# songweige/rich-text-to-image

Hardware: NVIDIA H100
Metric: denoising steps/sec (higher is better)
Workload: dtype f16

## Files before the change

### rich-text-to-image_b200/csrc/gemm_geglu.cu

```cuda
#include "ptx.cuh"
#include "rtti_internal.h"

namespace rtti {
namespace gg {
constexpr int BM = 128, BN = 128, BK = 64;
constexpr int STAGES = 4;
constexpr int A_TILE = BM * BK * 2;
constexpr int B_TILE = 2 * BN * BK * 2;
constexpr int STAGE = A_TILE + B_TILE;
constexpr int OFF_BAR = STAGES * STAGE;
constexpr int SMEM_BYTES = OFF_BAR + 64 + 1024;
constexpr int THREADS = 256;
}

struct GegluParams {
  const __half* bias;
  __half* y;
  int M, N, K;
  int n_blocks, k_blocks;
};

__device__ __forceinline__ float gelu_erf(float x) { return 0.5f * x * (1.f + erff(x * 0.70710678118654752f)); }

__global__ void __launch_bounds__(gg::THREADS, 1)
ff_geglu_kernel(const __grid_constant__ CUtensorMap tm_a, const __grid_constant__ CUtensorMap tm_b,
                const __grid_constant__ GegluParams p) {
  using namespace gg;
  extern __shared__ uint8_t smem_raw[];
  uint8_t* smem = reinterpret_cast<uint8_t*>((reinterpret_cast<uintptr_t>(smem_raw) + 1023) & ~uintptr_t(1023));
  uint64_t* full = reinterpret_cast<uint64_t*>(smem + OFF_BAR);

  const int tid = threadIdx.x, wg = tid >> 7, w = (tid >> 5) & 3, lane = tid & 31;
  const int m0 = (blockIdx.x / p.n_blocks) * BM, n0 = (blockIdx.x % p.n_blocks) * BN;

  auto load = [&](int kb) {
    const int s = kb % STAGES;
    uint8_t* st = smem + s * STAGE;
    mbar_expect_tx(&full[s], STAGE);
    tma_load_2d(st, &tm_a, &full[s], kb * BK, m0);
    tma_load_2d(st + A_TILE, &tm_b, &full[s], kb * BK, n0);
    tma_load_2d(st + A_TILE + B_TILE / 2, &tm_b, &full[s], kb * BK, p.N + n0);
  };
  if (tid == 0) {
    tma_prefetch_desc(&tm_a); tma_prefetch_desc(&tm_b);
    for (int i = 0; i < STAGES; ++i) mbar_init(&full[i], 1);
    mbar_fence_init();
    for (int kb = 0; kb < STAGES && kb < p.k_blocks; ++kb) load(kb);
  }
  __syncthreads();

  const uint32_t sbase = smem_u32(smem);
  float v[64], g[64];
  for (int kb = 0; kb < p.k_blocks; ++kb) {
    const int s = kb % STAGES;
    const uint32_t aa = sbase + s * STAGE + wg * 64 * 128;
    const uint32_t ba = sbase + s * STAGE + A_TILE;
    mbar_wait(&full[s], (kb / STAGES) & 1);
    wgmma_fence();
#pragma unroll
    for (int kk = 0; kk < BK / 16; ++kk) {
      const uint64_t da = wgmma_desc_sw128(aa + kk * 32, 16, 1024);
      const uint32_t acc = (kb > 0 || kk > 0) ? 1u : 0u;
      wgmma_ss<128>(v, da, wgmma_desc_sw128(ba + kk * 32, 16, 1024), acc);
      wgmma_ss<128>(g, da, wgmma_desc_sw128(ba + B_TILE / 2 + kk * 32, 16, 1024), acc);
    }
    wgmma_commit();
    wgmma_wait_all<64>(v);
    pin_regs<64>(g);
    __syncthreads();
    if (tid == 0 && kb + STAGES < p.k_blocks) load(kb + STAGES);
  }

  const int r0 = m0 + 64 * wg + 16 * w + (lane >> 2), r1 = r0 + 8;
  const int cq = 2 * (lane & 3);
#pragma unroll
  for (int i = 0; i < 16; ++i) {
    const int col = n0 + 8 * i + cq;
    float2 bv = make_float2(0.f, 0.f), bg = make_float2(0.f, 0.f);
    if (p.bias != nullptr) {
      bv = __half22float2(*reinterpret_cast<const __half2*>(p.bias + col));
      bg = __half22float2(*reinterpret_cast<const __half2*>(p.bias + p.N + col));
    }
    if (r0 < p.M)
      *reinterpret_cast<__half2*>(p.y + static_cast<size_t>(r0) * p.N + col) =
          __floats2half2_rn((v[4 * i] + bv.x) * gelu_erf(g[4 * i] + bg.x), (v[4 * i + 1] + bv.y) * gelu_erf(g[4 * i + 1] + bg.y));
    if (r1 < p.M)
      *reinterpret_cast<__half2*>(p.y + static_cast<size_t>(r1) * p.N + col) =
          __floats2half2_rn((v[4 * i + 2] + bv.x) * gelu_erf(g[4 * i + 2] + bg.x), (v[4 * i + 3] + bv.y) * gelu_erf(g[4 * i + 3] + bg.y));
  }
}

static int make_2d_map(CUtensorMap* m, const void* ptr, long long rows, long long cols, long long row_stride_elems,
                       int box_rows) {
  cuuint64_t dims[2] = {(cuuint64_t)cols, (cuuint64_t)rows};
  cuuint64_t strides[1] = {(cuuint64_t)row_stride_elems * 2};
  cuuint32_t box[2] = {64, (cuuint32_t)box_rows};
  cuuint32_t estr[2] = {1, 1};
  return encode_tiled_f16(m, ptr, 2, dims, strides, box, estr);
}

}

using namespace rtti;

extern "C" int rtti_ff_geglu_fwd(const void* x, const void* w, const void* bias, void* y, long long m, int n, int k,
                                 void* stream) {
  if (!x || !w || !y) return RTTI_ERR_ARG;
  if (m < 1 || n < 1 || k < 1) return RTTI_ERR_ARG;
  if (n % gg::BN != 0 || k % gg::BK != 0) return RTTI_ERR_SHAPE;
  if (((uintptr_t)x | (uintptr_t)w | (uintptr_t)y | (uintptr_t)bias) & 15) return RTTI_ERR_ALIGN;
  int rc = rtti_arch_ok();
  if (rc != RTTI_OK) return rc;
  CUtensorMap ta, tb;
  if ((rc = make_2d_map(&ta, x, m, k, k, gg::BM)) != RTTI_OK) return rc;
  if ((rc = make_2d_map(&tb, w, 2LL * n, k, k, gg::BN)) != RTTI_OK) return rc;
  static const bool configured =
      cudaFuncSetAttribute(ff_geglu_kernel, cudaFuncAttributeMaxDynamicSharedMemorySize, gg::SMEM_BYTES) == cudaSuccess;
  if (!configured) return RTTI_ERR_CUDA;
  GegluParams p{};
  p.bias = (const __half*)bias; p.y = (__half*)y; p.M = (int)m; p.N = n; p.K = k;
  p.n_blocks = n / gg::BN; p.k_blocks = k / gg::BK;
  const long long tiles = ((m + gg::BM - 1) / gg::BM) * p.n_blocks;
  if (tiles > 0x7fffffffLL) return RTTI_ERR_SHAPE;
  ff_geglu_kernel<<<(unsigned)tiles, gg::THREADS, gg::SMEM_BYTES, (cudaStream_t)stream>>>(ta, tb, p);
  return cudaGetLastError() == cudaSuccess ? RTTI_OK : RTTI_ERR_CUDA;
}
```

### rich-text-to-image_b200/csrc/ptx.cuh

```cuda
#pragma once
#include <cuda.h>
#include <cuda_fp16.h>
#include <cuda_runtime.h>
#include <stdint.h>

namespace rtti {

__device__ __forceinline__ uint32_t smem_u32(const void* p) {
  return static_cast<uint32_t>(__cvta_generic_to_shared(p));
}

__device__ __forceinline__ void mbar_init(uint64_t* bar, uint32_t count) {
  asm volatile("mbarrier.init.shared::cta.b64 [%0], %1;\n" ::"r"(smem_u32(bar)), "r"(count));
}
__device__ __forceinline__ void mbar_fence_init() {
  asm volatile("fence.mbarrier_init.release.cluster;\n" ::: "memory");
}
__device__ __forceinline__ void mbar_expect_tx(uint64_t* bar, uint32_t bytes) {
  asm volatile("mbarrier.arrive.expect_tx.shared::cta.b64 _, [%0], %1;\n" ::"r"(smem_u32(bar)),
               "r"(bytes)
               : "memory");
}
__device__ __forceinline__ void mbar_arrive(uint64_t* bar) {
  asm volatile("mbarrier.arrive.shared::cta.b64 _, [%0];\n" ::"r"(smem_u32(bar)) : "memory");
}
__device__ __forceinline__ void mbar_wait(uint64_t* bar, uint32_t parity) {
  asm volatile(
      "{\n\t.reg .pred P1;\n\t"
      "WAIT_LOOP:\n\t"
      "mbarrier.try_wait.parity.shared::cta.b64 P1, [%0], %1;\n\t"
      "@P1 bra.uni WAIT_DONE;\n\t"
      "bra.uni WAIT_LOOP;\n\t"
      "WAIT_DONE:\n\t}\n" ::"r"(smem_u32(bar)),
      "r"(parity)
      : "memory");
}

__device__ __forceinline__ void tma_prefetch_desc(const CUtensorMap* m) {
  asm volatile("prefetch.tensormap [%0];\n" ::"l"(reinterpret_cast<uint64_t>(m)) : "memory");
}
__device__ __forceinline__ void tma_load_4d(void* smem_dst, const CUtensorMap* m, uint64_t* bar, int c0,
                                            int c1, int c2, int c3) {
  asm volatile(
      "cp.async.bulk.tensor.4d.shared::cluster.global.mbarrier::complete_tx::bytes"
      " [%0], [%1, {%3, %4, %5, %6}], [%2];\n" ::"r"(smem_u32(smem_dst)),
      "l"(reinterpret_cast<uint64_t>(m)), "r"(smem_u32(bar)), "r"(c0), "r"(c1), "r"(c2), "r"(c3)
      : "memory");
}
__device__ __forceinline__ void tma_store_4d(const CUtensorMap* m, const void* smem_src, int c0, int c1,
                                             int c2, int c3) {
  asm volatile(
      "cp.async.bulk.tensor.4d.global.shared::cta.bulk_group [%0, {%2, %3, %4, %5}], [%1];\n" ::"l"(
          reinterpret_cast<uint64_t>(m)),
      "r"(smem_u32(smem_src)), "r"(c0), "r"(c1), "r"(c2), "r"(c3)
      : "memory");
}
__device__ __forceinline__ void tma_store_commit() { asm volatile("cp.async.bulk.commit_group;\n" ::: "memory"); }
__device__ __forceinline__ void tma_store_wait_read() {
  asm volatile("cp.async.bulk.wait_group.read 0;\n" ::: "memory");
}
__device__ __forceinline__ void tma_store_wait_all() {
  asm volatile("cp.async.bulk.wait_group 0;\n" ::: "memory");
}
__device__ __forceinline__ void fence_proxy_async_smem() {
  asm volatile("fence.proxy.async.shared::cta;\n" ::: "memory");
}

__device__ __forceinline__ void tma_load_2d(void* smem_dst, const CUtensorMap* m, uint64_t* bar, int c0, int c1) {
  asm volatile(
      "cp.async.bulk.tensor.2d.shared::cluster.global.mbarrier::complete_tx::bytes"
      " [%0], [%1, {%3, %4}], [%2];\n" ::"r"(smem_u32(smem_dst)),
      "l"(reinterpret_cast<uint64_t>(m)), "r"(smem_u32(bar)), "r"(c0), "r"(c1)
      : "memory");
}

__device__ __forceinline__ uint64_t wgmma_desc_sw128(uint32_t smem_addr, uint32_t lbo_bytes, uint32_t sbo_bytes) {
  uint64_t d = 0;
  d |= static_cast<uint64_t>((smem_addr & 0x3FFFF) >> 4);
  d |= static_cast<uint64_t>((lbo_bytes >> 4) & 0x3FFF) << 16;
  d |= static_cast<uint64_t>((sbo_bytes >> 4) & 0x3FFF) << 32;
  d |= static_cast<uint64_t>(1) << 62;
  return d;
}

__device__ __forceinline__ void wgmma_fence() { asm volatile("wgmma.fence.sync.aligned;\n" ::: "memory"); }
__device__ __forceinline__ void wgmma_commit() { asm volatile("wgmma.commit_group.sync.aligned;\n" ::: "memory"); }
template <int N>
__device__ __forceinline__ void wgmma_wait_all(float* d) {
  asm volatile("wgmma.wait_group.sync.aligned 0;\n" ::: "memory");
#pragma unroll
  for (int i = 0; i < N; ++i) asm volatile("" : "+f"(d[i])::"memory");
}
template <int N>
__device__ __forceinline__ void pin_regs(float* d) {
#pragma unroll
  for (int i = 0; i < N; ++i) asm volatile("" : "+f"(d[i])::"memory");
}

template <int N> __device__ __forceinline__ void wgmma_ss(float* d, uint64_t da, uint64_t db, uint32_t acc);
template <int N> __device__ __forceinline__ void wgmma_rs_tb(float* d, const uint32_t* a, uint64_t db, uint32_t acc);
template <> __device__ __forceinline__ void wgmma_ss<64>(float* d, uint64_t da, uint64_t db, uint32_t acc) {
  asm volatile(
      "{\n\t.reg .pred p;\n\tsetp.ne.b32 p, %34, 0;\n\t"
      "wgmma.mma_async.sync.aligned.m64n64k16.f32.f16.f16 {%0, %1, %2, %3, %4, %5, %6, %7, %8, %9, %10, %11, %12, %13, %14, %15, %16, %17, %18, %19, %20, %21, %22, %23, %24, %25, %26, %27, %28, %29, %30, %31}, %32, %33, p, 1, 1, 0, 0;\n\t}\n"
      : "+f"(d[0]), "+f"(d[1]), "+f"(d[2]), "+f"(d[3]), "+f"(d[4]), "+f"(d[5]), "+f"(d[6]), "+f"(d[7]), "+f"(d[8]), "+f"(d[9]), "+f"(d[10]), "+f"(d[11]), "+f"(d[12]), "+f"(d[13]), "+f"(d[14]), "+f"(d[15]), "+f"(d[16]), "+f"(d[17]), "+f"(d[18]), "+f"(d[19]), "+f"(d[20]), "+f"(d[21]), "+f"(d[22]), "+f"(d[23]), "+f"(d[24]), "+f"(d[25]), "+f"(d[26]), "+f"(d[27]), "+f"(d[28]), "+f"(d[29]), "+f"(d[30]), "+f"(d[31])
      : "l"(da), "l"(db), "r"(acc));
}

template <> __device__ __forceinline__ void wgmma_ss<80>(float* d, uint64_t da, uint64_t db, uint32_t acc) {
  asm volatile(
      "{\n\t.reg .pred p;\n\tsetp.ne.b32 p, %42, 0;\n\t"
      "wgmma.mma_async.sync.aligned.m64n80k16.f32.f16.f16 {%0, %1, %2, %3, %4, %5, %6, %7, %8, %9, %10, %11, %12, %13, %14, %15, %16, %17, %18, %19, %20, %21, %22, %23, %24, %25, %26, %27, %28, %29, %30, %31, %32, %33, %34, %35, %36, %37, %38, %39}, %40, %41, p, 1, 1, 0, 0;\n\t}\n"
      : "+f"(d[0]), "+f"(d[1]), "+f"(d[2]), "+f"(d[3]), "+f"(d[4]), "+f"(d[5]), "+f"(d[6]), "+f"(d[7]), "+f"(d[8]), "+f"(d[9]), "+f"(d[10]), "+f"(d[11]), "+f"(d[12]), "+f"(d[13]), "+f"(d[14]), "+f"(d[15]), "+f"(d[16]), "+f"(d[17]), "+f"(d[18]), "+f"(d[19]), "+f"(d[20]), "+f"(d[21]), "+f"(d[22]), "+f"(d[23]), "+f"(d[24]), "+f"(d[25]), "+f"(d[26]), "+f"(d[27]), "+f"(d[28]), "+f"(d[29]), "+f"(d[30]), "+f"(d[31]), "+f"(d[32]), "+f"(d[33]), "+f"(d[34]), "+f"(d[35]), "+f"(d[36]), "+f"(d[37]), "+f"(d[38]), "+f"(d[39])
      : "l"(da), "l"(db), "r"(acc));
}

template <> __device__ __forceinline__ void wgmma_ss<128>(float* d, uint64_t da, uint64_t db, uint32_t acc) {
  asm volatile(
      "{\n\t.reg .pred p;\n\tsetp.ne.b32 p, %66, 0;\n\t"
      "wgmma.mma_async.sync.aligned.m64n128k16.f32.f16.f16 {%0, %1, %2, %3, %4, %5, %6, %7, %8, %9, %10, %11, %12, %13, %14, %15, %16, %17, %18, %19, %20, %21, %22, %23, %24, %25, %26, %27, %28, %29, %30, %31, %32, %33, %34, %35, %36, %37, %38, %39, %40, %41, %42, %43, %44, %45, %46, %47, %48, %49, %50, %51, %52, %53, %54, %55, %56, %57, %58, %59, %60, %61, %62, %63}, %64, %65, p, 1, 1, 0, 0;\n\t}\n"
      : "+f"(d[0]), "+f"(d[1]), "+f"(d[2]), "+f"(d[3]), "+f"(d[4]), "+f"(d[5]), "+f"(d[6]), "+f"(d[7]), "+f"(d[8]), "+f"(d[9]), "+f"(d[10]), "+f"(d[11]), "+f"(d[12]), "+f"(d[13]), "+f"(d[14]), "+f"(d[15]), "+f"(d[16]), "+f"(d[17]), "+f"(d[18]), "+f"(d[19]), "+f"(d[20]), "+f"(d[21]), "+f"(d[22]), "+f"(d[23]), "+f"(d[24]), "+f"(d[25]), "+f"(d[26]), "+f"(d[27]), "+f"(d[28]), "+f"(d[29]), "+f"(d[30]), "+f"(d[31]), "+f"(d[32]), "+f"(d[33]), "+f"(d[34]), "+f"(d[35]), "+f"(d[36]), "+f"(d[37]), "+f"(d[38]), "+f"(d[39]), "+f"(d[40]), "+f"(d[41]), "+f"(d[42]), "+f"(d[43]), "+f"(d[44]), "+f"(d[45]), "+f"(d[46]), "+f"(d[47]), "+f"(d[48]), "+f"(d[49]), "+f"(d[50]), "+f"(d[51]), "+f"(d[52]), "+f"(d[53]), "+f"(d[54]), "+f"(d[55]), "+f"(d[56]), "+f"(d[57]), "+f"(d[58]), "+f"(d[59]), "+f"(d[60]), "+f"(d[61]), "+f"(d[62]), "+f"(d[63])
      : "l"(da), "l"(db), "r"(acc));
}

template <> __device__ __forceinline__ void wgmma_rs_tb<64>(float* d, const uint32_t* a, uint64_t db, uint32_t acc) {
  asm volatile(
      "{\n\t.reg .pred p;\n\tsetp.ne.b32 p, %37, 0;\n\t"
      "wgmma.mma_async.sync.aligned.m64n64k16.f32.f16.f16 {%0, %1, %2, %3, %4, %5, %6, %7, %8, %9, %10, %11, %12, %13, %14, %15, %16, %17, %18, %19, %20, %21, %22, %23, %24, %25, %26, %27, %28, %29, %30, %31}, {%32, %33, %34, %35}, %36, p, 1, 1, 1;\n\t}\n"
      : "+f"(d[0]), "+f"(d[1]), "+f"(d[2]), "+f"(d[3]), "+f"(d[4]), "+f"(d[5]), "+f"(d[6]), "+f"(d[7]), "+f"(d[8]), "+f"(d[9]), "+f"(d[10]), "+f"(d[11]), "+f"(d[12]), "+f"(d[13]), "+f"(d[14]), "+f"(d[15]), "+f"(d[16]), "+f"(d[17]), "+f"(d[18]), "+f"(d[19]), "+f"(d[20]), "+f"(d[21]), "+f"(d[22]), "+f"(d[23]), "+f"(d[24]), "+f"(d[25]), "+f"(d[26]), "+f"(d[27]), "+f"(d[28]), "+f"(d[29]), "+f"(d[30]), "+f"(d[31])
      : "r"(a[0]), "r"(a[1]), "r"(a[2]), "r"(a[3]), "l"(db), "r"(acc));
}

__device__ __forceinline__ float ex2_approx(float x) {
  float y;
  asm("ex2.approx.ftz.f32 %0, %1;\n" : "=f"(y) : "f"(x));
  return y;
}
__device__ __forceinline__ uint32_t pack_half2(float lo, float hi) {
  __half2 h = __floats2half2_rn(lo, hi);
  return *reinterpret_cast<uint32_t*>(&h);
}

}
```

### rich-text-to-image_b200/unet.py

```python
import math
from dataclasses import dataclass, field
from typing import Dict, List, Optional, Tuple

import torch
import torch.nn as nn
import torch.nn.functional as F

from . import ops

FEATURE_INJECT_RESNET = "up_blocks.1.resnets.1"


@dataclass
class UNetConfig:
    sample_size: int = 64
    in_channels: int = 4
    out_channels: int = 4
    down_block_types: Tuple[str, ...] = ("CrossAttnDownBlock2D", "CrossAttnDownBlock2D", "CrossAttnDownBlock2D", "DownBlock2D")
    up_block_types: Tuple[str, ...] = ("UpBlock2D", "CrossAttnUpBlock2D", "CrossAttnUpBlock2D", "CrossAttnUpBlock2D")
    block_out_channels: Tuple[int, ...] = (320, 640, 1280, 1280)
    layers_per_block: int = 2
    transformer_layers_per_block: Tuple[int, ...] = (1, 1, 1, 1)
    attention_head_dim: Tuple[int, ...] = (8, 8, 8, 8)
    cross_attention_dim: int = 768
    use_linear_projection: bool = False
    addition_embed_type: Optional[str] = None
    addition_time_embed_dim: Optional[int] = None
    projection_class_embeddings_input_dim: Optional[int] = None
    norm_num_groups: int = 32
    norm_eps: float = 1e-5
    flip_sin_to_cos: bool = True
    freq_shift: int = 0

    @staticmethod
    def sd15():
        return UNetConfig()

    @staticmethod
    def sdxl():
        return UNetConfig(sample_size=128, down_block_types=("DownBlock2D", "CrossAttnDownBlock2D", "CrossAttnDownBlock2D"),
                          up_block_types=("CrossAttnUpBlock2D", "CrossAttnUpBlock2D", "UpBlock2D"),
                          block_out_channels=(320, 640, 1280), transformer_layers_per_block=(1, 2, 10),
                          attention_head_dim=(5, 10, 20), cross_attention_dim=2048, use_linear_projection=True,
                          addition_embed_type="text_time", addition_time_embed_dim=256,
                          projection_class_embeddings_input_dim=2816)

    @staticmethod
    def from_dict(d):
        keys = UNetConfig.__dataclass_fields__.keys()
        kw = {k: (tuple(v) if isinstance(v, list) else v) for k, v in d.items() if k in keys}
        n = len(kw.get("block_out_channels", (0,) * 4))
        for k in ("transformer_layers_per_block", "attention_head_dim"):
            if k in kw and isinstance(kw[k], int):
                kw[k] = (kw[k],) * n
        return UNetConfig(**kw)


class TokenMapAccumulator:

    def __init__(self, cross_layers, self_layers=None, start_after=10, sd_overwrite_bug=False,
                 self_resolutions=(32,)):
        self.cross_layers = set(cross_layers)
        self.self_layers = None if self_layers is None else set(self_layers)
        self.start_after = start_after
        self.sd_overwrite_bug = sd_overwrite_bug
        self.self_resolutions = None if self_resolutions is None else set(self_resolutions)
        self.selfattn_maps: Dict[str, torch.Tensor] = {}
        self.crossattn_maps: Dict[str, torch.Tensor] = {}
        self.n_maps: Dict[str, int] = {}

    def tick(self, name):
        self.n_maps[name] = self.n_maps.get(name, 0) + 1
        return self.n_maps[name] > self.start_after

    def cross_target(self, name, n_q, n_k, device):
        if not self.tick(name) or name not in self.cross_layers:
            return None
        if name not in self.crossattn_maps:
            self.crossattn_maps[name] = torch.zeros(1, n_q, n_k, dtype=torch.float32, device=device)
        return self.crossattn_maps[name]

    def self_target(self, name, n_q, device):
        if not self.tick(name):
            return None
        if self.self_layers is not None and name not in self.self_layers:
            return None
        if self.self_resolutions is not None and int(round(math.sqrt(n_q))) not in self.self_resolutions:
            return None
        if name not in self.selfattn_maps:
            self.selfattn_maps[name] = torch.zeros(1, n_q, n_q, dtype=torch.float32, device=device)
        elif self.sd_overwrite_bug and name not in self.crossattn_maps:
            self.selfattn_maps[name].zero_()
        return self.selfattn_maps[name]


class CrossKVCache:

    def __init__(self):
        self.kv: Dict[str, torch.Tensor] = {}


@dataclass
class RegionControl:
    qk_src: Optional[List[int]] = None
    feature_src: Optional[List[int]] = None
    feature_idx: Optional[torch.Tensor] = None
    word_pos: Optional[torch.Tensor] = None
    font_size: Optional[torch.Tensor] = None
    fs_batch_mask: int = 0
    capture: Optional[TokenMapAccumulator] = None
    capture_row: int = 1
    kv_cache: Optional[CrossKVCache] = None
    remote: Optional[object] = None


def _f16(t):
    return t.to(torch.float16)


class GroupNormCL(nn.Module):

    def __init__(self, groups, channels, eps):
        super().__init__()
        self.groups, self.eps = groups, eps
        self.weight = nn.Parameter(torch.ones(channels))
        self.bias = nn.Parameter(torch.zeros(channels))

    def forward(self, x, silu, chan_bias=None):
        return ops.groupnorm_silu(x, self.weight, self.bias, self.groups, self.eps, silu, chan_bias=chan_bias)


class LayerNormCL(nn.Module):
    def __init__(self, channels, eps=1e-5):
        super().__init__()
        self.eps = eps
        self.weight = nn.Parameter(torch.ones(channels))
        self.bias = nn.Parameter(torch.zeros(channels))

    def forward(self, x):
        return ops.layernorm(x, self.weight, self.bias, self.eps)


class Conv2dCL(nn.Conv2d):

    def forward_cl(self, x, H, W, with_bias=True):
        B = x.shape[0]
        x4 = x.view(B, H, W, -1).permute(0, 3, 1, 2)
        y = F.conv2d(x4, self.weight, self.bias if with_bias else None, self.stride, self.padding)
        Ho, Wo = y.shape[2], y.shape[3]
        y = y.permute(0, 2, 3, 1)
        if not y.is_contiguous():
            y = y.contiguous()
        return y.reshape(B, Ho * Wo, -1), Ho, Wo


class Attention(nn.Module):

    def __init__(self, query_dim, cross_attention_dim, heads):
        super().__init__()
        self.heads = heads
        self.is_cross = cross_attention_dim is not None
        kv_dim = cross_attention_dim if self.is_cross else query_dim
        self.to_q = nn.Linear(query_dim, query_dim, bias=False)
        self.to_k = nn.Linear(kv_dim, query_dim, bias=False)
        self.to_v = nn.Linear(kv_dim, query_dim, bias=False)
        self.to_out = nn.ModuleList([nn.Linear(query_dim, query_dim)])
        self._fused = None

    def fused_weight(self):
        ver = (self.to_k.weight._version, self.to_v.weight._version, self.to_q.weight._version,
               self.to_k.weight.data_ptr(), self.to_k.weight.dtype)
        if self._fused is None or self._fused[0] != ver:
            ws = [self.to_k.weight, self.to_v.weight] if self.is_cross else [self.to_q.weight, self.to_k.weight, self.to_v.weight]
            self._fused = (ver, torch.cat([w.detach() for w in ws], 0).contiguous())
        return self._fused[1]


class BasicTransformerBlock(nn.Module):
    def __init__(self, dim, heads, cross_attention_dim):
        super().__init__()
        self.norm1 = LayerNormCL(dim)
        self.attn1 = Attention(dim, None, heads)
        self.norm2 = LayerNormCL(dim)
        self.attn2 = Attention(dim, cross_attention_dim, heads)
        self.norm3 = LayerNormCL(dim)
        self.ff = nn.Module()
        self.ff.net = nn.ModuleList([nn.Module(), nn.Identity(), nn.Linear(dim * 4, dim)])
        self.ff.net[0].proj = nn.Linear(dim, dim * 8)

    def forward(self, h, n, ctx, ctrl: RegionControl, name):
        B, T, C = h.shape
        heads = self.attn1.heads
        cap = ctrl.capture
        rem = ctrl.remote
        if rem is not None and rem.is_dst:
            k0 = rem.n_own
            w3 = self.attn1.fused_weight()
            o = torch.empty(B, T, C, dtype=h.dtype, device=h.device)
            if k0:
                qkv = F.linear(n[:k0], w3)
                ops.attention(qkv[..., :C], qkv[..., C:2 * C], qkv[..., 2 * C:], heads, out=o[:k0])
            v = F.linear(n[k0:], w3[2 * C:])
            rqk = rem.wait(T, 2 * C)
            ops.attention(rqk[..., :C], rqk[..., C:], v, heads, qk_src=[0] * (B - k0), out=o[k0:])
        else:
            qkv = F.linear(n, self.attn1.fused_weight())
            q, k, v = qkv[..., :C], qkv[..., C:2 * C], qkv[..., 2 * C:]
            if rem is not None and rem.is_src:
                rem.push(qkv[rem.d_index, :, :2 * C])
            tgt = cap.self_target(name + ".attn1", T, h.device) if cap is not None else None
            lse = torch.empty(B, heads, T, dtype=torch.float32, device=h.device) if tgt is not None else None
            o = ops.attention(q, k, v, heads, qk_src=ctrl.qk_src, lse=lse)
            if tgt is not None:
                r = ctrl.capture_row
                ops.attn_probs_mean_accum(q[r], k[r], lse[r], tgt[0], heads)
        a = F.linear(o, self.attn1.to_out[0].weight)
        h, n = ops.add_bias_layernorm(a, h, self.attn1.to_out[0].bias, self.norm2.weight, self.norm2.bias, self.norm2.eps)
        q = F.linear(n, self.attn2.to_q.weight)
        kv = None
        key = name + ".attn2"
        if ctrl.kv_cache is not None:
            kv = ctrl.kv_cache.kv.get(key)
        if kv is None:
            kv = F.linear(ctx, self.attn2.fused_weight())
            if ctrl.kv_cache is not None:
                ctrl.kv_cache.kv[key] = kv
        ck, cv = kv[..., :C], kv[..., C:]
        pbar, slots = None, None
        if cap is not None:
            pbar = cap.cross_target(key, T, ctx.shape[1], h.device)
            if pbar is not None:
                slots = [-1] * B
                slots[ctrl.capture_row] = 0
        o = ops.attention(q, ck, cv, heads, word_pos=ctrl.word_pos, font_size=ctrl.font_size,
                          fs_batch_mask=ctrl.fs_batch_mask, pbar_accum=pbar, cap_slot=slots)
        a = F.linear(o, self.attn2.to_out[0].weight)
        h, n = ops.add_bias_layernorm(a, h, self.attn2.to_out[0].bias, self.norm3.weight, self.norm3.bias, self.norm3.eps)
        proj = self.ff.net[0].proj
        if ops.FUSED_FF_GEGLU and C % 64 == 0:
            g = ops.ff_geglu(n, proj.weight, proj.bias)
        else:
            g = ops.geglu(F.linear(n, proj.weight, proj.bias))
        a = F.linear(g, self.ff.net[2].weight)
        if rem is not None and rem.is_src:
            rem.join()
            del qkv
        return h, a, self.ff.net[2].bias


class Transformer2DModel(nn.Module):
    def __init__(self, channels, heads, layers, cross_attention_dim, groups, use_linear_projection):
        super().__init__()
        self.use_linear_projection = use_linear_projection
        self.norm = GroupNormCL(groups, channels, 1e-6)
        if use_linear_projection:
            self.proj_in = nn.Linear(channels, channels)
            self.proj_out = nn.Linear(channels, channels)
        else:
            self.proj_in = nn.Conv2d(channels, channels, 1)
            self.proj_out = nn.Conv2d(channels, channels, 1)
        self.transformer_blocks = nn.ModuleList([BasicTransformerBlock(channels, heads, cross_attention_dim) for _ in range(layers)])

    def _proj(self, mod, x):
        w = mod.weight if self.use_linear_projection else mod.weight.view(mod.weight.shape[0], -1)
        return F.linear(x, w, mod.bias)

    def forward(self, x, ctx, ctrl, name):
        h = self.norm(x, silu=False)
        h = self._proj(self.proj_in, h)
        blocks = self.transformer_blocks
        n = blocks[0].norm1(h)
        for i, blk in enumerate(blocks):
            h, a, bias = blk(h, n, ctx, ctrl, f"{name}.transformer_blocks.{i}")
            if i + 1 < len(blocks):
                nxt = blocks[i + 1].norm1
                h, n = ops.add_bias_layernorm(a, h, bias, nxt.weight, nxt.bias, nxt.eps)
            else:
                h = ops.add_bias_f16(h, a, bias, out=a)
        w = self.proj_out.weight if self.use_linear_projection else self.proj_out.weight.view(self.proj_out.weight.shape[0], -1)
        y = F.linear(h, w)
        return ops.add_bias_f16(x, y, self.proj_out.bias, out=y)


class ResnetBlock2D(nn.Module):
    def __init__(self, cin, cout, temb_ch, groups, eps):
        super().__init__()
        self.norm1 = GroupNormCL(groups, cin, eps)
        self.conv1 = Conv2dCL(cin, cout, 3, padding=1)
        self.time_emb_proj = nn.Linear(temb_ch, cout)
        self.norm2 = GroupNormCL(groups, cout, eps)
        self.conv2 = Conv2dCL(cout, cout, 3, padding=1)
        self.conv_shortcut = nn.Conv2d(cin, cout, 1) if cin != cout else None

    def forward(self, x, H, W, temb_act, feature_idx=None, remote=None):
        h = self.norm1(x, silu=True)
        h, _, _ = self.conv1.forward_cl(h, H, W, with_bias=False)
        t = F.linear(temb_act, self.time_emb_proj.weight, self.time_emb_proj.bias + self.conv1.bias)
        h = self.norm2(h, silu=True, chan_bias=t.contiguous())
        h, _, _ = self.conv2.forward_cl(h, H, W, with_bias=False)
        if remote is not None and remote.is_src:
            remote.push(h[remote.d_index])
            remote.join()
        if remote is not None and remote.is_dst:
            f = remote.wait(h.shape[1], h.shape[2])
            h = torch.cat([h[:remote.n_own], f.expand(h.shape[0] - remote.n_own, -1, -1)], 0)
        elif feature_idx is not None:
            h = h.index_select(0, feature_idx)
        if self.conv_shortcut is not None:
            x = F.linear(x, self.conv_shortcut.weight.view(self.conv_shortcut.weight.shape[0], -1), self.conv_shortcut.bias)
        return ops.add_bias_f16(x, h, self.conv2.bias, out=h)


class Downsample2D(nn.Module):
    def __init__(self, ch):
        super().__init__()
        self.conv = Conv2dCL(ch, ch, 3, stride=2, padding=1)


class Upsample2D(nn.Module):
    def __init__(self, ch):
        super().__init__()
        self.conv = Conv2dCL(ch, ch, 3, padding=1)

    def forward(self, x, H, W):
        B, _, C = x.shape
        x = x.view(B, H, 1, W, 1, C).expand(B, H, 2, W, 2, C).reshape(B, 4 * H * W, C)
        return self.conv.forward_cl(x, 2 * H, 2 * W)


class _Block(nn.Module):
    pass


class UNet2DConditionModel(nn.Module):
    def __init__(self, cfg: UNetConfig):
        super().__init__()
        self.config = cfg
        self.in_channels = cfg.in_channels
        boc = cfg.block_out_channels
        temb = boc[0] * 4
        g, eps = cfg.norm_num_groups, cfg.norm_eps
        self.conv_in = Conv2dCL(cfg.in_channels, boc[0], 3, padding=1)
        self.time_embedding = nn.Module()
        self.time_embedding.linear_1 = nn.Linear(boc[0], temb)
        self.time_embedding.linear_2 = nn.Linear(temb, temb)
        if cfg.addition_embed_type == "text_time":
            self.add_embedding = nn.Module()
            self.add_embedding.linear_1 = nn.Linear(cfg.projection_class_embeddings_input_dim, temb)
            self.add_embedding.linear_2 = nn.Linear(temb, temb)
        self.down_blocks = nn.ModuleList()
        out_c = boc[0]
        for i, typ in enumerate(cfg.down_block_types):
            in_c, out_c = out_c, boc[i]
            blk = _Block()
            blk.has_cross_attention = typ == "CrossAttnDownBlock2D"
            if blk.has_cross_attention:
                blk.attentions = nn.ModuleList([
                    Transformer2DModel(out_c, cfg.attention_head_dim[i], cfg.transformer_layers_per_block[i],
                                       cfg.cross_attention_dim, g, cfg.use_linear_projection)
                    for _ in range(cfg.layers_per_block)])
            blk.resnets = nn.ModuleList([ResnetBlock2D(in_c if l == 0 else out_c, out_c, temb, g, eps)
                                         for l in range(cfg.layers_per_block)])
            if i != len(boc) - 1:
                blk.downsamplers = nn.ModuleList([Downsample2D(out_c)])
            else:
                blk.downsamplers = None
            self.down_blocks.append(blk)
        self.mid_block = _Block()
        self.mid_block.attentions = nn.ModuleList([
            Transformer2DModel(boc[-1], cfg.attention_head_dim[-1], cfg.transformer_layers_per_block[-1],
                               cfg.cross_attention_dim, g, cfg.use_linear_projection)])
        self.mid_block.resnets = nn.ModuleList([ResnetBlock2D(boc[-1], boc[-1], temb, g, eps) for _ in range(2)])
        self.up_blocks = nn.ModuleList()
        rev = list(reversed(boc))
        rev_heads = list(reversed(cfg.attention_head_dim))
        rev_layers = list(reversed(cfg.transformer_layers_per_block))
        out_c = rev[0]
        for i, typ in enumerate(cfg.up_block_types):
            prev, out_c = out_c, rev[i]
            in_c = rev[min(i + 1, len(boc) - 1)]
            n = cfg.layers_per_block + 1
            blk = _Block()
            blk.has_cross_attention = typ == "CrossAttnUpBlock2D"
            if blk.has_cross_attention:
                blk.attentions = nn.ModuleList([
                    Transformer2DModel(out_c, rev_heads[i], rev_layers[i], cfg.cross_attention_dim, g, cfg.use_linear_projection)
                    for _ in range(n)])
            blk.resnets = nn.ModuleList([
                ResnetBlock2D((prev if l == 0 else out_c) + (in_c if l == n - 1 else out_c), out_c, temb, g, eps)
                for l in range(n)])
            blk.upsamplers = nn.ModuleList([Upsample2D(out_c)]) if i != len(boc) - 1 else None
            self.up_blocks.append(blk)
        self.conv_norm_out = GroupNormCL(g, boc[0], eps)
        self.conv_out = Conv2dCL(boc[0], cfg.out_channels, 3, padding=1)

    def injection_layout(self, H, W):
        out = []

        def attn(tr, H, W):
            C = tr.proj_in.weight.shape[0]
            out.extend([(H * W, 2 * C)] * len(tr.transformer_blocks))

        for i, blk in enumerate(self.down_blocks):
            for l in range(len(blk.resnets)):
                if blk.has_cross_attention:
                    attn(blk.attentions[l], H, W)
            if blk.downsamplers is not None:
                H, W = (H + 1) // 2, (W + 1) // 2
        attn(self.mid_block.attentions[0], H, W)
        for i, blk in enumerate(self.up_blocks):
            for l, res in enumerate(blk.resnets):
                if f"up_blocks.{i}.resnets.{l}" == FEATURE_INJECT_RESNET:
                    out.append((H * W, res.conv2.weight.shape[0]))
                if blk.has_cross_attention:
                    attn(blk.attentions[l], H, W)
            if blk.upsamplers is not None:
                H, W = 2 * H, 2 * W
        return out

    def finalize(self, device="cuda"):
        self.to(device=device, dtype=torch.float16)
        for m in self.modules():
            if isinstance(m, nn.Conv2d) and m.kernel_size != (1, 1):
                m.weight.data = m.weight.data.contiguous(memory_format=torch.channels_last)
        self.requires_grad_(False)
        return self.eval()

    def init_synthetic(self, seed=0):
        g = torch.Generator(device=self.conv_in.weight.device).manual_seed(seed)
        for name, p in self.named_parameters():
            if p.dim() >= 2:
                fan_in = p[0].numel()
                p.data.copy_(torch.randn(p.shape, generator=g, device=p.device, dtype=torch.float32) / math.sqrt(fan_in))
            elif name.endswith("weight"):
                p.data.fill_(1.0)
            else:
                p.data.copy_(0.05 * torch.randn(p.shape, generator=g, device=p.device, dtype=torch.float32))
        return self

    def _timestep_embedding(self, t, dim, device):
        half = dim // 2
        exponent = -math.log(10000) * torch.arange(half, dtype=torch.float32, device=device) / (half - self.config.freq_shift)
        emb = t[:, None].float() * torch.exp(exponent)[None, :]
        emb = torch.cat([torch.sin(emb), torch.cos(emb)], dim=-1)
        if self.config.flip_sin_to_cos:
            emb = torch.cat([emb[:, half:], emb[:, :half]], dim=-1)
        return emb

    def forward(self, sample, timestep, encoder_hidden_states, added_cond_kwargs=None, ctrl: Optional[RegionControl] = None,
                return_dict=True, **unused):
        cfg = self.config
        ctrl = ctrl or RegionControl()
        dev = sample.device
        B, _, H, W = sample.shape
        t = torch.as_tensor(timestep, device=dev)
        if t.dim() == 0:
            t = t[None]
        t = t.expand(B)
        mlp = lambda m, x: F.linear(F.silu(F.linear(x, m.linear_1.weight, m.linear_1.bias)), m.linear_2.weight, m.linear_2.bias)
        emb = mlp(self.time_embedding, _f16(self._timestep_embedding(t, cfg.block_out_channels[0], dev)))
        if cfg.addition_embed_type == "text_time":
            time_ids = added_cond_kwargs["time_ids"].to(dev)
            te = self._timestep_embedding(time_ids.flatten(), cfg.addition_time_embed_dim, dev)
            te = te.reshape(time_ids.shape[0], -1)
            if te.shape[0] != B:
                te = te[:1].expand(B, -1)
            add = torch.cat([_f16(added_cond_kwargs["text_embeds"]), _f16(te)], dim=-1)
            emb = emb + mlp(self.add_embedding, add)
        temb_act = F.silu(emb)
        ctx = _f16(encoder_hidden_states).contiguous()
        feat_idx = ctrl.feature_idx
        if feat_idx is None and ctrl.feature_src is not None:
            feat_idx = torch.as_tensor(ctrl.feature_src, device=dev)

        x = _f16(sample).permute(0, 2, 3, 1).contiguous().view(B, H * W, -1)
        h, H, W = self.conv_in.forward_cl(x, H, W)
        skips = [(h, H, W)]
        for i, blk in enumerate(self.down_blocks):
            for l, res in enumerate(blk.resnets):
                h = res(h, H, W, temb_act)
                if blk.has_cross_attention:
                    h = blk.attentions[l](h, ctx, ctrl, f"down_blocks.{i}.attentions.{l}")
                skips.append((h, H, W))
            if blk.downsamplers is not None:
                h, H, W = blk.downsamplers[0].conv.forward_cl(h, H, W)
                skips.append((h, H, W))
        h = self.mid_block.resnets[0](h, H, W, temb_act)
        h = self.mid_block.attentions[0](h, ctx, ctrl, "mid_block.attentions.0")
        h = self.mid_block.resnets[1](h, H, W, temb_act)
        for i, blk in enumerate(self.up_blocks):
            for l, res in enumerate(blk.resnets):
                s, _, _ = skips.pop()
                h = torch.cat([h, s], dim=-1)
                rname = f"up_blocks.{i}.resnets.{l}"
                inj = rname == FEATURE_INJECT_RESNET
                h = res(h, H, W, temb_act, feat_idx if inj else None, ctrl.remote if inj else None)
                if blk.has_cross_attention:
                    h = blk.attentions[l](h, ctx, ctrl, f"up_blocks.{i}.attentions.{l}")
            if blk.upsamplers is not None:
                h, H, W = blk.upsamplers[0](h, H, W)
        h = self.conv_norm_out(h, silu=True)
        h, H, W = self.conv_out.forward_cl(h, H, W)
        out = h.view(B, H, W, -1).permute(0, 3, 1, 2).contiguous()
        return {"sample": out} if return_dict else (out,)
```

Measured before the change: 4.810.

## Warp-specialize persistent GEGLU GEMM and skip redundant QK projections in self-attention

The GEGLU feed-forward GEMM becomes a persistent, warp-specialized kernel. One producer warpgroup issues TMA loads through full/empty mbarriers while two consumer warpgroups each run m64n256 wgmma over both value and gate halves, with register reallocation via setmaxnreg. Tiles are swizzled in groups along M for L2 reuse, and outputs are staged in shared memory and written with TMA stores. Separately, the UNet self-attention path now computes only V for batch rows whose Q/K come from an earlier row and reuses that row's QK. This cuts GEMM work but adds control logic and shape assumptions.

```diff
diff --git a/rich-text-to-image_b200/csrc/gemm_geglu.cu b/rich-text-to-image_b200/csrc/gemm_geglu.cu
--- a/rich-text-to-image_b200/csrc/gemm_geglu.cu
+++ b/rich-text-to-image_b200/csrc/gemm_geglu.cu
@@ -5,89 +5,128 @@
 namespace gg {
 constexpr int BM = 128, BN = 128, BK = 64;
 constexpr int STAGES = 4;
+constexpr int GROUP_M = 8;
 constexpr int A_TILE = BM * BK * 2;
 constexpr int B_TILE = 2 * BN * BK * 2;
 constexpr int STAGE = A_TILE + B_TILE;
-constexpr int OFF_BAR = STAGES * STAGE;
-constexpr int SMEM_BYTES = OFF_BAR + 64 + 1024;
-constexpr int THREADS = 256;
+constexpr int OUT_BOX = 64 * 64 * 2;
+constexpr int OFF_OUT = STAGES * STAGE;
+constexpr int OFF_BAR = OFF_OUT + 2 * 2 * OUT_BOX;
+constexpr int SMEM_BYTES = OFF_BAR + 2 * STAGES * 8 + 1024;
+constexpr int THREADS = 384;
+constexpr int PRODUCER_REGS = 40, CONSUMER_REGS = 232;
 }
 
 struct GegluParams {
   const __half* bias;
-  __half* y;
   int M, N, K;
-  int n_blocks, k_blocks;
+  int m_blocks, n_blocks, k_blocks, tiles;
 };
 
 __device__ __forceinline__ float gelu_erf(float x) { return 0.5f * x * (1.f + erff(x * 0.70710678118654752f)); }
 
+__device__ __forceinline__ void tile_origin(const GegluParams& p, int tile, int& m0, int& n0) {
+  const int per_group = gg::GROUP_M * p.n_blocks;
+  const int first_m = (tile / per_group) * gg::GROUP_M;
+  const int gm = min(p.m_blocks - first_m, gg::GROUP_M);
+  const int r = tile % per_group;
+  m0 = (first_m + r % gm) * gg::BM;
+  n0 = (r / gm) * gg::BN;
+}
+
 __global__ void __launch_bounds__(gg::THREADS, 1)
 ff_geglu_kernel(const __grid_constant__ CUtensorMap tm_a, const __grid_constant__ CUtensorMap tm_b,
-                const __grid_constant__ GegluParams p) {
+                const __grid_constant__ CUtensorMap tm_y, const __grid_constant__ GegluParams p) {
   using namespace gg;
   extern __shared__ uint8_t smem_raw[];
   uint8_t* smem = reinterpret_cast<uint8_t*>((reinterpret_cast<uintptr_t>(smem_raw) + 1023) & ~uintptr_t(1023));
   uint64_t* full = reinterpret_cast<uint64_t*>(smem + OFF_BAR);
+  uint64_t* empty = full + STAGES;
 
   const int tid = threadIdx.x, wg = tid >> 7, w = (tid >> 5) & 3, lane = tid & 31;
-  const int m0 = (blockIdx.x / p.n_blocks) * BM, n0 = (blockIdx.x % p.n_blocks) * BN;
-
-  auto load = [&](int kb) {
-    const int s = kb % STAGES;
-    uint8_t* st = smem + s * STAGE;
-    mbar_expect_tx(&full[s], STAGE);
-    tma_load_2d(st, &tm_a, &full[s], kb * BK, m0);
-    tma_load_2d(st + A_TILE, &tm_b, &full[s], kb * BK, n0);
-    tma_load_2d(st + A_TILE + B_TILE / 2, &tm_b, &full[s], kb * BK, p.N + n0);
-  };
   if (tid == 0) {
-    tma_prefetch_desc(&tm_a); tma_prefetch_desc(&tm_b);
-    for (int i = 0; i < STAGES; ++i) mbar_init(&full[i], 1);
+    tma_prefetch_desc(&tm_a); tma_prefetch_desc(&tm_b); tma_prefetch_desc(&tm_y);
+    for (int i = 0; i < STAGES; ++i) { mbar_init(&full[i], 1); mbar_init(&empty[i], 8); }
     mbar_fence_init();
-    for (int kb = 0; kb < STAGES && kb < p.k_blocks; ++kb) load(kb);
   }
   __syncthreads();
 
-  const uint32_t sbase = smem_u32(smem);
-  float v[64], g[64];
-  for (int kb = 0; kb < p.k_blocks; ++kb) {
-    const int s = kb % STAGES;
-    const uint32_t aa = sbase + s * STAGE + wg * 64 * 128;
-    const uint32_t ba = sbase + s * STAGE + A_TILE;
-    mbar_wait(&full[s], (kb / STAGES) & 1);
-    wgmma_fence();
-#pragma unroll
-    for (int kk = 0; kk < BK / 16; ++kk) {
-      const uint64_t da = wgmma_desc_sw128(aa + kk * 32, 16, 1024);
-      const uint32_t acc = (kb > 0 || kk > 0) ? 1u : 0u;
-      wgmma_ss<128>(v, da, wgmma_desc_sw128(ba + kk * 32, 16, 1024), acc);
-      wgmma_ss<128>(g, da, wgmma_desc_sw128(ba + B_TILE / 2 + kk * 32, 16, 1024), acc);
+  if (wg == 0) {
+    setmaxnreg_dec<PRODUCER_REGS>();
+    if (tid != 0) return;
+    int it = 0;
+    for (int tile = blockIdx.x; tile < p.tiles; tile += gridDim.x) {
+      int m0, n0;
+      tile_origin(p, tile, m0, n0);
+      for (int kb = 0; kb < p.k_blocks; ++kb, ++it) {
+        const int s = it % STAGES;
+        uint8_t* st = smem + s * STAGE;
+        mbar_wait(&empty[s], ((it / STAGES) & 1) ^ 1);
+        mbar_expect_tx(&full[s], STAGE);
+        tma_load_2d(st, &tm_a, &full[s], kb * BK, m0);
+        tma_load_2d(st + A_TILE, &tm_b, &full[s], kb * BK, n0);
+        tma_load_2d(st + A_TILE + B_TILE / 2, &tm_b, &full[s], kb * BK, p.N + n0);
+      }
     }
-    wgmma_commit();
-    wgmma_wait_all<64>(v);
-    pin_regs<64>(g);
-    __syncthreads();
-    if (tid == 0 && kb + STAGES < p.k_blocks) load(kb + STAGES);
+    return;
   }
 
-  const int r0 = m0 + 64 * wg + 16 * w + (lane >> 2), r1 = r0 + 8;
+  setmaxnreg_inc<CONSUMER_REGS>();
+  const int c = wg - 1;
+  const uint32_t sbase = smem_u32(smem);
+  uint8_t* out = smem + OFF_OUT + c * 2 * OUT_BOX;
+  const int r0 = 16 * w + (lane >> 2), r1 = r0 + 8;
   const int cq = 2 * (lane & 3);
+  float acc[128];
+  int it = 0;
+  for (int tile = blockIdx.x; tile < p.tiles; tile += gridDim.x) {
+    int m0, n0;
+    tile_origin(p, tile, m0, n0);
+    for (int kb = 0; kb < p.k_blocks; ++kb, ++it) {
+      const int s = it % STAGES;
+      const uint32_t aa = sbase + s * STAGE + c * 64 * 128;
+      const uint32_t ba = sbase + s * STAGE + A_TILE;
+      mbar_wait(&full[s], (it / STAGES) & 1);
+      wgmma_fence();
 #pragma unroll
-  for (int i = 0; i < 16; ++i) {
-    const int col = n0 + 8 * i + cq;
-    float2 bv = make_float2(0.f, 0.f), bg = make_float2(0.f, 0.f);
-    if (p.bias != nullptr) {
-      bv = __half22float2(*reinterpret_cast<const __half2*>(p.bias + col));
-      bg = __half22float2(*reinterpret_cast<const __half2*>(p.bias + p.N + col));
+      for (int kk = 0; kk < BK / 16; ++kk)
+        wgmma_ss<256>(acc, wgmma_desc_sw128(aa + kk * 32, 16, 1024), wgmma_desc_sw128(ba + kk * 32, 16, 1024),
+                      (kb > 0 || kk > 0) ? 1u : 0u);
+      wgmma_commit();
+      wgmma_wait<1>();
+      if (kb > 0 && lane == 0) mbar_arrive(&empty[(it - 1) % STAGES]);
     }
-    if (r0 < p.M)
-      *reinterpret_cast<__half2*>(p.y + static_cast<size_t>(r0) * p.N + col) =
-          __floats2half2_rn((v[4 * i] + bv.x) * gelu_erf(g[4 * i] + bg.x), (v[4 * i + 1] + bv.y) * gelu_erf(g[4 * i + 1] + bg.y));
-    if (r1 < p.M)
-      *reinterpret_cast<__half2*>(p.y + static_cast<size_t>(r1) * p.N + col) =
-          __floats2half2_rn((v[4 * i + 2] + bv.x) * gelu_erf(g[4 * i + 2] + bg.x), (v[4 * i + 3] + bv.y) * gelu_erf(g[4 * i + 3] + bg.y));
+    wgmma_wait<0>();
+    pin_regs<128>(acc);
+    if (lane == 0) mbar_arrive(&empty[(it - 1) % STAGES]);
+
+    if (tid % 128 == 0) tma_store_wait_read();
+    named_barrier(1 + c, 128);
+#pragma unroll
+    for (int i = 0; i < 16; ++i) {
+      const int col = n0 + 8 * i + cq;
+      float2 bv = make_float2(0.f, 0.f), bg = make_float2(0.f, 0.f);
+      if (p.bias != nullptr) {
+        bv = __half22float2(*reinterpret_cast<const __half2*>(p.bias + col));
+        bg = __half22float2(*reinterpret_cast<const __half2*>(p.bias + p.N + col));
+      }
+      const float* v = acc + 4 * i;
+      const float* g = acc + 64 + 4 * i;
+      uint8_t* box = out + (i >> 3) * OUT_BOX + cq * 2;
+      *reinterpret_cast<uint32_t*>(box + r0 * 128 + (((i & 7) ^ (r0 & 7)) << 4)) =
+          pack_half2((v[0] + bv.x) * gelu_erf(g[0] + bg.x), (v[1] + bv.y) * gelu_erf(g[1] + bg.y));
+      *reinterpret_cast<uint32_t*>(box + r1 * 128 + (((i & 7) ^ (r1 & 7)) << 4)) =
+          pack_half2((v[2] + bv.x) * gelu_erf(g[2] + bg.x), (v[3] + bv.y) * gelu_erf(g[3] + bg.y));
+    }
+    fence_proxy_async_smem();
+    named_barrier(1 + c, 128);
+    if (tid % 128 == 0 && m0 + 64 * c < p.M) {
+      tma_store_2d(&tm_y, out, n0, m0 + 64 * c);
+      tma_store_2d(&tm_y, out + OUT_BOX, n0 + 64, m0 + 64 * c);
+      tma_store_commit();
+    }
   }
+  if (tid % 128 == 0) tma_store_wait_all();
 }
 
 static int make_2d_map(CUtensorMap* m, const void* ptr, long long rows, long long cols, long long row_stride_elems,
@@ -111,17 +150,26 @@
   if (((uintptr_t)x | (uintptr_t)w | (uintptr_t)y | (uintptr_t)bias) & 15) return RTTI_ERR_ALIGN;
   int rc = rtti_arch_ok();
   if (rc != RTTI_OK) return rc;
-  CUtensorMap ta, tb;
+  CUtensorMap ta, tb, ty;
   if ((rc = make_2d_map(&ta, x, m, k, k, gg::BM)) != RTTI_OK) return rc;
   if ((rc = make_2d_map(&tb, w, 2LL * n, k, k, gg::BN)) != RTTI_OK) return rc;
+  if ((rc = make_2d_map(&ty, y, m, n, n, 64)) != RTTI_OK) return rc;
   static const bool configured =
       cudaFuncSetAttribute(ff_geglu_kernel, cudaFuncAttributeMaxDynamicSharedMemorySize, gg::SMEM_BYTES) == cudaSuccess;
   if (!configured) return RTTI_ERR_CUDA;
+  static const int n_sm = [] {
+    int dev = 0, v = 132;
+    cudaGetDevice(&dev);
+    cudaDeviceGetAttribute(&v, cudaDevAttrMultiProcessorCount, dev);
+    return v;
+  }();
+  const long long m_blocks = (m + gg::BM - 1) / gg::BM;
+  const long long tiles = m_blocks * (n / gg::BN);
+  if (m > 0x7fffffffLL || tiles > 0x7fffffffLL) return RTTI_ERR_SHAPE;
   GegluParams p{};
-  p.bias = (const __half*)bias; p.y = (__half*)y; p.M = (int)m; p.N = n; p.K = k;
-  p.n_blocks = n / gg::BN; p.k_blocks = k / gg::BK;
-  const long long tiles = ((m + gg::BM - 1) / gg::BM) * p.n_blocks;
-  if (tiles > 0x7fffffffLL) return RTTI_ERR_SHAPE;
-  ff_geglu_kernel<<<(unsigned)tiles, gg::THREADS, gg::SMEM_BYTES, (cudaStream_t)stream>>>(ta, tb, p);
+  p.bias = (const __half*)bias; p.M = (int)m; p.N = n; p.K = k;
+  p.m_blocks = (int)m_blocks; p.n_blocks = n / gg::BN; p.k_blocks = k / gg::BK; p.tiles = (int)tiles;
+  const unsigned grid = (unsigned)(tiles < n_sm ? tiles : n_sm);
+  ff_geglu_kernel<<<grid, gg::THREADS, gg::SMEM_BYTES, (cudaStream_t)stream>>>(ta, tb, ty, p);
   return cudaGetLastError() == cudaSuccess ? RTTI_OK : RTTI_ERR_CUDA;
 }
diff --git a/rich-text-to-image_b200/csrc/ptx.cuh b/rich-text-to-image_b200/csrc/ptx.cuh
--- a/rich-text-to-image_b200/csrc/ptx.cuh
+++ b/rich-text-to-image_b200/csrc/ptx.cuh
@@ -74,6 +74,20 @@
       : "memory");
 }
 
+__device__ __forceinline__ void tma_store_2d(const CUtensorMap* m, const void* smem_src, int c0, int c1) {
+  asm volatile(
+      "cp.async.bulk.tensor.2d.global.shared::cta.bulk_group [%0, {%2, %3}], [%1];\n" ::"l"(
+          reinterpret_cast<uint64_t>(m)),
+      "r"(smem_u32(smem_src)), "r"(c0), "r"(c1)
+      : "memory");
+}
+
+template <int N> __device__ __forceinline__ void setmaxnreg_dec() { asm volatile("setmaxnreg.dec.sync.aligned.u32 %0;\n" ::"n"(N)); }
+template <int N> __device__ __forceinline__ void setmaxnreg_inc() { asm volatile("setmaxnreg.inc.sync.aligned.u32 %0;\n" ::"n"(N)); }
+__device__ __forceinline__ void named_barrier(int id, int threads) {
+  asm volatile("bar.sync %0, %1;\n" ::"r"(id), "r"(threads) : "memory");
+}
+
 __device__ __forceinline__ uint64_t wgmma_desc_sw128(uint32_t smem_addr, uint32_t lbo_bytes, uint32_t sbo_bytes) {
   uint64_t d = 0;
   d |= static_cast<uint64_t>((smem_addr & 0x3FFFF) >> 4);
@@ -90,6 +104,10 @@
   asm volatile("wgmma.wait_group.sync.aligned 0;\n" ::: "memory");
 #pragma unroll
   for (int i = 0; i < N; ++i) asm volatile("" : "+f"(d[i])::"memory");
+}
+template <int N>
+__device__ __forceinline__ void wgmma_wait() {
+  asm volatile("wgmma.wait_group.sync.aligned %0;\n" ::"n"(N) : "memory");
 }
 template <int N>
 __device__ __forceinline__ void pin_regs(float* d) {
@@ -123,6 +141,14 @@
       : "l"(da), "l"(db), "r"(acc));
 }
 
+template <> __device__ __forceinline__ void wgmma_ss<256>(float* d, uint64_t da, uint64_t db, uint32_t acc) {
+  asm volatile(
+      "{\n\t.reg .pred p;\n\tsetp.ne.b32 p, %130, 0;\n\t"
+      "wgmma.mma_async.sync.aligned.m64n256k16.f32.f16.f16 {%0, %1, %2, %3, %4, %5, %6, %7, %8, %9, %10, %11, %12, %13, %14, %15, %16, %17, %18, %19, %20, %21, %22, %23, %24, %25, %26, %27, %28, %29, %30, %31, %32, %33, %34, %35, %36, %37, %38, %39, %40, %41, %42, %43, %44, %45, %46, %47, %48, %49, %50, %51, %52, %53, %54, %55, %56, %57, %58, %59, %60, %61, %62, %63, %64, %65, %66, %67, %68, %69, %70, %71, %72, %73, %74, %75, %76, %77, %78, %79, %80, %81, %82, %83, %84, %85, %86, %87, %88, %89, %90, %91, %92, %93, %94, %95, %96, %97, %98, %99, %100, %101, %102, %103, %104, %105, %106, %107, %108, %109, %110, %111, %112, %113, %114, %115, %116, %117, %118, %119, %120, %121, %122, %123, %124, %125, %126, %127}, %128, %129, p, 1, 1, 0, 0;\n\t}\n"
+      : "+f"(d[0]), "+f"(d[1]), "+f"(d[2]), "+f"(d[3]), "+f"(d[4]), "+f"(d[5]), "+f"(d[6]), "+f"(d[7]), "+f"(d[8]), "+f"(d[9]), "+f"(d[10]), "+f"(d[11]), "+f"(d[12]), "+f"(d[13]), "+f"(d[14]), "+f"(d[15]), "+f"(d[16]), "+f"(d[17]), "+f"(d[18]), "+f"(d[19]), "+f"(d[20]), "+f"(d[21]), "+f"(d[22]), "+f"(d[23]), "+f"(d[24]), "+f"(d[25]), "+f"(d[26]), "+f"(d[27]), "+f"(d[28]), "+f"(d[29]), "+f"(d[30]), "+f"(d[31]), "+f"(d[32]), "+f"(d[33]), "+f"(d[34]), "+f"(d[35]), "+f"(d[36]), "+f"(d[37]), "+f"(d[38]), "+f"(d[39]), "+f"(d[40]), "+f"(d[41]), "+f"(d[42]), "+f"(d[43]), "+f"(d[44]), "+f"(d[45]), "+f"(d[46]), "+f"(d[47]), "+f"(d[48]), "+f"(d[49]), "+f"(d[50]), "+f"(d[51]), "+f"(d[52]), "+f"(d[53]), "+f"(d[54]), "+f"(d[55]), "+f"(d[56]), "+f"(d[57]), "+f"(d[58]), "+f"(d[59]), "+f"(d[60]), "+f"(d[61]), "+f"(d[62]), "+f"(d[63]), "+f"(d[64]), "+f"(d[65]), "+f"(d[66]), "+f"(d[67]), "+f"(d[68]), "+f"(d[69]), "+f"(d[70]), "+f"(d[71]), "+f"(d[72]), "+f"(d[73]), "+f"(d[74]), "+f"(d[75]), "+f"(d[76]), "+f"(d[77]), "+f"(d[78]), "+f"(d[79]), "+f"(d[80]), "+f"(d[81]), "+f"(d[82]), "+f"(d[83]), "+f"(d[84]), "+f"(d[85]), "+f"(d[86]), "+f"(d[87]), "+f"(d[88]), "+f"(d[89]), "+f"(d[90]), "+f"(d[91]), "+f"(d[92]), "+f"(d[93]), "+f"(d[94]), "+f"(d[95]), "+f"(d[96]), "+f"(d[97]), "+f"(d[98]), "+f"(d[99]), "+f"(d[100]), "+f"(d[101]), "+f"(d[102]), "+f"(d[103]), "+f"(d[104]), "+f"(d[105]), "+f"(d[106]), "+f"(d[107]), "+f"(d[108]), "+f"(d[109]), "+f"(d[110]), "+f"(d[111]), "+f"(d[112]), "+f"(d[113]), "+f"(d[114]), "+f"(d[115]), "+f"(d[116]), "+f"(d[117]), "+f"(d[118]), "+f"(d[119]), "+f"(d[120]), "+f"(d[121]), "+f"(d[122]), "+f"(d[123]), "+f"(d[124]), "+f"(d[125]), "+f"(d[126]), "+f"(d[127])
+      : "l"(da), "l"(db), "r"(acc));
+}
+
 template <> __device__ __forceinline__ void wgmma_rs_tb<64>(float* d, const uint32_t* a, uint64_t db, uint32_t acc) {
   asm volatile(
       "{\n\t.reg .pred p;\n\tsetp.ne.b32 p, %37, 0;\n\t"
diff --git a/rich-text-to-image_b200/unet.py b/rich-text-to-image_b200/unet.py
--- a/rich-text-to-image_b200/unet.py
+++ b/rich-text-to-image_b200/unet.py
@@ -118,6 +118,18 @@
     return t.to(torch.float16)
 
 
+def _self_sourced_prefix(qk_src, batch):
+    if qk_src is None:
+        return batch
+    k0 = 0
+    while k0 < batch and qk_src[k0] == k0:
+        k0 += 1
+    suffix = qk_src[k0:]
+    if suffix and max(suffix) < k0 and max(suffix) - min(suffix) < batch - k0:
+        return k0
+    return batch
+
+
 class GroupNormCL(nn.Module):
 
     def __init__(self, groups, channels, eps):
@@ -195,14 +207,24 @@
         rem = ctrl.remote
         if rem is not None and rem.is_dst:
             k0 = rem.n_own
+        else:
+            k0 = _self_sourced_prefix(ctrl.qk_src, B) if cap is None else B
+        if k0 < B:
             w3 = self.attn1.fused_weight()
             o = torch.empty(B, T, C, dtype=h.dtype, device=h.device)
             if k0:
                 qkv = F.linear(n[:k0], w3)
+                if rem is not None and rem.is_src:
+                    rem.push(qkv[rem.d_index, :, :2 * C])
                 ops.attention(qkv[..., :C], qkv[..., C:2 * C], qkv[..., 2 * C:], heads, out=o[:k0])
             v = F.linear(n[k0:], w3[2 * C:])
-            rqk = rem.wait(T, 2 * C)
-            ops.attention(rqk[..., :C], rqk[..., C:], v, heads, qk_src=[0] * (B - k0), out=o[k0:])
+            if rem is not None and rem.is_dst:
+                qk, src = rem.wait(T, 2 * C), [0] * (B - k0)
+            else:
+                lo = min(ctrl.qk_src[k0:])
+                src = [s - lo for s in ctrl.qk_src[k0:]]
+                qk = qkv[lo:lo + max(src) + 1, :, :2 * C]
+            ops.attention(qk[..., :C], qk[..., C:], v, heads, qk_src=src, out=o[k0:])
         else:
             qkv = F.linear(n, self.attn1.fused_weight())
             q, k, v = qkv[..., :C], qkv[..., C:2 * C], qkv[..., 2 * C:]
```

Result: faster. 5.034, median of 6 (+4.7%).
